# seanwood/gcc-nmf

Measured on AMD Instinct MI355X. Metric: stereo frames/sec (1024-FFT, K=1024, 100 NMF iters), higher is better.
Workload: dtype f32; 1 GPU; HBM-resident (float32 samples in HBM -> separated float32 waveforms in HBM; the host-to-host rates are the host_to_host_* fields of a --full run): 64 x 10 s stereo @16 kHz synthetic mixtures per GPU (SURVEY 8d recipe), 1024-pt FFT hop 256 (F=513, T=622/file), K=1024, 100 KL-NMF iters, 128 TDOAs, 3 targets, independent dictionary per file; dictionary_size=1024, parallelism=file-sharded x1, no data-path collective

## Files before the change

gcc_nmf_amd/csrc/common.h:

```cpp
#pragma once
#include <hip/hip_runtime.h>
#include <stdint.h>

#define GCCNMF_OK 0
#define GCCNMF_ERR_ARG 1
#define GCCNMF_ERR_LAUNCH 2
#define GCCNMF_ERR_UNSUPPORTED 3

static inline int gccnmf_ceil_div(int a, int b) { return (a + b - 1) / b; }
static inline int gccnmf_round_up(int a, int b) { return gccnmf_ceil_div(a, b) * b; }

#define GCCNMF_CHECK_LAUNCH()                                   \
    do {                                                        \
        hipError_t e__ = hipGetLastError();                     \
        if (e__ != hipSuccess) return GCCNMF_ERR_LAUNCH;        \
    } while (0)

struct GccNmfPitches {
    int Fp, Kp, Np, Tp;
};

static inline GccNmfPitches gccnmf_make_pitches(int F, int T, int K) {
    GccNmfPitches p;
    p.Fp = gccnmf_round_up(F, 16);
    p.Kp = gccnmf_round_up(K, 64);
    p.Np = gccnmf_round_up(2 * T, 64);
    p.Tp = gccnmf_round_up(T, 64);
    return p;
}

#define GCCNMF_TUNE_KEYS 26
struct GccNmfTune {
    int v[GCCNMF_TUNE_KEYS];
};
extern thread_local GccNmfTune gccnmf_tune;
struct GccNmfCall {
    GccNmfCall();
    ~GccNmfCall();
};
#define GCCNMF_ENTER() GccNmfCall gccnmf_call_scope_
#define gccnmf_tune_ablate (gccnmf_tune.v[1])
#define gccnmf_tune_tile_policy (gccnmf_tune.v[2])
#define gccnmf_tune_dma (gccnmf_tune.v[3])
#define gccnmf_tune_ring (gccnmf_tune.v[4])
#define gccnmf_tune_wh_splits (gccnmf_tune.v[5])
#define gccnmf_tune_rht_splits (gccnmf_tune.v[6])
#define gccnmf_tune_exact_div (gccnmf_tune.v[7])
#define gccnmf_tune_shared_groups (gccnmf_tune.v[8])
#define gccnmf_tune_tail_split (gccnmf_tune.v[9])
#define gccnmf_tune_direct (gccnmf_tune.v[10])
#define gccnmf_tune_direct_tile (gccnmf_tune.v[11])
#define gccnmf_tune_direct_batch (gccnmf_tune.v[12])
#define gccnmf_tune_direct_depth (gccnmf_tune.v[13])
#define gccnmf_tune_short_updh (gccnmf_tune.v[14])
#define gccnmf_tune_fft_r16 (gccnmf_tune.v[15])
#define gccnmf_tune_fused_k12 (gccnmf_tune.v[16])
#define gccnmf_tune_fused_k34 (gccnmf_tune.v[17])
#define gccnmf_tune_persistent (gccnmf_tune.v[18])
#define gccnmf_tune_prefetch (gccnmf_tune.v[19])
#define gccnmf_tune_wide_update_w (gccnmf_tune.v[20])
#define gccnmf_tune_chain (gccnmf_tune.v[21])
#define gccnmf_tune_chain_solo (gccnmf_tune.v[22])
#define gccnmf_tune_chain_rag (gccnmf_tune.v[23])
#define gccnmf_tune_chain_chunk (gccnmf_tune.v[24])
#define gccnmf_tune_chain_fault (gccnmf_tune.v[25])
```

gcc_nmf_amd/csrc/gcc.hip:

```cpp
#include "gemm_ring.h"
#include "ratio.h"
#include "spatial.h"
#include "angular_nl.h"
#include "atom_tdoa.h"
#include "source_count.h"
#include "../../include/gccnmf_hip.h"


static bool gcc_small_launch(int batch, int M, int N, int Kd) {
    if (!gccnmf_tune_ring || !gccnmf_ring_supports(Kd) || gccnmf_tune_tile_policy == 1) return false;
    if (gccnmf_tune_tile_policy == 2) return true;
    return (long)batch * gccnmf_ceil_div(M, 512) * gccnmf_ceil_div(N, 64) < 256;
}

__global__ __launch_bounds__(256) void ang_mean_kernel(const float* __restrict__ ang, int T, int D, int Dp, int Tp,
                                                       double* __restrict__ mean_ang) {
    __shared__ double red[256];
    const int b = blockIdx.x / D, d = blockIdx.x - b * D;
    const float* row = ang + ((long)b * Dp + d) * Tp;
    double s = 0.0;
    for (int t = threadIdx.x; t < T; t += 256) s += (double)row[t];
    red[threadIdx.x] = s;
    __syncthreads();
    for (int w = 128; w > 0; w >>= 1) {
// ... 150 lines not shown
        const float* sin_row = trig + ((long)Fp + f) * Dp;
        int4 tau;
        if (TRACKS) tau = *(const int4*)(tdoa_idx + ((long)b * S + i) * Tp + t);
        else tau.x = tau.y = tau.z = tau.w = tdoa_idx[(long)b * S + i];
        const bool absent = COUNTED && tau.x < 0;
        tau.x = tau.x < 0 ? 0 : (tau.x >= D ? D - 1 : tau.x);
        tau.y = tau.y < 0 ? 0 : (tau.y >= D ? D - 1 : tau.y);
        tau.z = tau.z < 0 ? 0 : (tau.z >= D ? D - 1 : tau.z);
        tau.w = tau.w < 0 ? 0 : (tau.w >= D ? D - 1 : tau.w);
        out = gcc_steer4(cr, ci, make_float4(cos_row[tau.x], cos_row[tau.y], cos_row[tau.z], cos_row[tau.w]),
                         make_float4(sin_row[tau.x], sin_row[tau.y], sin_row[tau.z], sin_row[tau.w]));
        if (absent) out.x = out.y = out.z = out.w = __builtin_nanf("");
        if (t + 1 >= T) out.y = 0.f;
        if (t + 2 >= T) out.z = 0.f;
        if (t + 3 >= T) out.w = 0.f;
    }
    *(float4*)(P + ((long)b * Fp + f) * ((long)S * Tp) + col) = out;
}

__global__ __launch_bounds__(256) void gcc_argmax_kernel(const float* __restrict__ scores, int K, int Kp, int T, int Tp, int S,
                                                         unsigned char* __restrict__ argmax) {
    const int t = 4 * (blockIdx.x * 256 + threadIdx.x);
    const int k = blockIdx.y, b = blockIdx.z;
    if (t >= Tp) return;
    unsigned char best[4] = {0, 0, 0, 0};
    if (k < K && t < T) {
        const float* row = scores + ((long)b * Kp + k) * ((long)S * Tp) + t;
        float bv[4] = {0.f, 0.f, 0.f, 0.f};
        bool have[4] = {false, false, false, false};
        for (int i = 0; i < S; ++i) {
            const float4 v4 = *(const float4*)(row + (long)i * Tp);
            const float v[4] = {v4.x, v4.y, v4.z, v4.w};
#pragma unroll
            for (int j = 0; j < 4; ++j) {
                if (v[j] != v[j]) continue;
                if (!have[j] || v[j] > bv[j]) {
                    bv[j] = v[j];
                    best[j] = (unsigned char)i;
                    have[j] = true;
                }
            }
        }
#pragma unroll
        for (int j = 1; j < 4; ++j)
            if (t + j >= T) best[j] = 0;
    }
    *(uchar4*)(argmax + ((long)b * Kp + k) * Tp + t) = make_uchar4(best[0], best[1], best[2], best[3]);
}

__global__ __launch_bounds__(256) void gcc_coherence_kernel(const float2* __restrict__ X, int Fp, int T, int Tp,
                                                            float* __restrict__ CC) {
    const int t = blockIdx.x * 256 + threadIdx.x;
    const int f = blockIdx.y, b = blockIdx.z;
    if (t >= T) return;
    const long plane = (long)Fp * Tp;
    const float2 xl = X[(long)b * 2 * plane + (long)f * Tp + t];
    const float2 xr = X[(long)b * 2 * plane + plane + (long)f * Tp + t];
    const float aL = hypotf(xl.x, xl.y), aR = hypotf(xr.x, xr.y);
    float re = xl.x * xr.x + xl.y * xr.y, im = xl.y * xr.x - xl.x * xr.y;
    if (aL > 0.f && aR > 0.f) {
        re = re / aL / aR;
        im = im / aL / aR;
    } else {
        re = 0.f;
        im = 0.f;
    }
    float* Cb = CC + (long)b * 2 * plane + (long)f * Tp + t;
    Cb[0] = re;
    Cb[plane] = im;
}

__global__ __launch_bounds__(256) void gcc_magnitude_kernel(const float2* __restrict__ X, int Fp, int T, int Tp, int Np,
                                                            float* __restrict__ V) {
    const int t = blockIdx.x * 256 + threadIdx.x;
    const int f = blockIdx.y, b = blockIdx.z >> 1, c = blockIdx.z & 1;
    if (t >= T) return;
    const float2 x = X[((long)b * 2 + c) * Fp * Tp + (long)f * Tp + t];
    V[(long)b * Fp * Np + (long)f * Np + c * T + t] = hypotf(x.x, x.y);
}

__global__ __launch_bounds__(256) void gcc_masked_h_kernel(const float* __restrict__ H, const unsigned char* __restrict__ argmax,
                                                           const float* __restrict__ masks, int K, int Kp, int T, int Tp, int Np,
                                                           int S, float* __restrict__ Hm) {
    const int col = 4 * (blockIdx.x * 256 + threadIdx.x);
    const int k = blockIdx.y, b = blockIdx.z;
    const int ncol = 2 * S * Tp;
    if (col >= ncol) return;
    const int ic = col / Tp, t = col - ic * Tp;
    const int i = ic >> 1, c = ic & 1;
    float4 out = make_float4(0.f, 0.f, 0.f, 0.f);
    if (k < K && t < T) {
        const float* h = H + ((long)b * Kp + k) * Np + c * T + t;
        float4 m;
        if (masks) {
            m = *(const float4*)(masks + (((long)b * S + i) * Kp + k) * Tp + t);
        } else {
            const uchar4 a = *(const uchar4*)(argmax + ((long)b * Kp + k) * Tp + t);
            m = make_float4(a.x == i ? 1.f : 0.f, a.y == i ? 1.f : 0.f, a.z == i ? 1.f : 0.f, a.w == i ? 1.f : 0.f);
        }
        out.x = h[0] * m.x;
        if (t + 1 < T) out.y = h[1] * m.y;
        if (t + 2 < T) out.z = h[2] * m.z;
        if (t + 3 < T) out.w = h[3] * m.w;
    }
    *(float4*)(Hm + ((long)b * Kp + k) * (long)ncol + col) = out;
}

int gccnmf_gemm_nn_store(const float* A, const float* B, float* C, int M, int N, int Kd, int lda, int ldb, int ldc, int batch, long sA,
                         long sB, long sC, hipStream_t s) {
    GemmArgs a = {};
    a.A = A; a.sA = sA; a.lda = lda; a.a_clamp = lda - 4;
    a.B = B; a.sB = sB; a.ldb = ldb; a.b_clamp = ldb - 4;
    a.M = M; a.N = N; a.Kd = Kd;
    a.batch = batch; a.xcd_affine = 0;
    a.C = C; a.sC = sC; a.ldc = ldc;
    if (gcc_small_launch(batch, a.M, a.N, a.Kd)) return gccnmf_launch_gemm_ring<false, false, EPI_STORE, false>(a, s);
    return (M > 128) ? gccnmf_launch_gemm<4, 1, false, false, EPI_STORE, false>(a, s) : gccnmf_launch_gemm<1, 4, false, false, EPI_STORE, false>(a, s);
}

extern "C" {

int gccnmf_angular_spectrogram(const float* CC, const float* trig, int F, int T, int D, int batch, float* ang,
                               double* mean_ang, void* stream) {
    GCCNMF_ENTER();
    const unsigned alpha_bits = ((unsigned)D & 0xffff0000u) | ((unsigned)batch >> 16);
    float nl_alpha = 0.f;
    if (alpha_bits) {
        __builtin_memcpy(&nl_alpha, &alpha_bits, sizeof(float));
        if (!gccnmf_nl_alpha_ok(nl_alpha)) return GCCNMF_ERR_ARG;
        D &= 0xffff;
        batch &= 0xffff;
    }
    if (!CC || !trig || !ang || F < 2 || T < 1 || D < 1 || batch < 1) return GCCNMF_ERR_ARG;
    hipStream_t s = (hipStream_t)stream;
    GccNmfPitches p = gccnmf_make_pitches(F, T, 1);
    const int Dp = gccnmf_round_up(D, 64);
    if (alpha_bits) {
        const int rc = gccnmf_launch_angular_nl(CC, trig, F, T, D, batch, nl_alpha, ang, s);
        if (rc) return rc;
        if (mean_ang) {
            hipLaunchKernelGGL(ang_mean_kernel, dim3(batch * D), dim3(256), 0, s, ang, T, D, Dp, p.Tp, mean_ang);
            GCCNMF_CHECK_LAUNCH();
        }
        return GCCNMF_OK;
    }
    GemmArgs a = {};
    a.A = trig; a.sA = 0; a.lda = Dp; a.a_clamp = Dp - 4;
    a.B = CC; a.sB = 2L * p.Fp * p.Tp; a.ldb = p.Tp; a.b_clamp = p.Tp - 4;
    a.M = D; a.N = T; a.Kd = 2 * p.Fp;
    a.batch = batch; a.xcd_affine = 0;
    a.C = ang; a.sC = (long)Dp * p.Tp; a.ldc = p.Tp;
    int rc;
    if (gcc_small_launch(batch, a.M, a.N, a.Kd)) rc = gccnmf_launch_gemm_ring<false, false, EPI_STORE, false>(a, s);
    else rc = (D > 128) ? gccnmf_launch_gemm<4, 1, false, false, EPI_STORE, false>(a, s)
                        : gccnmf_launch_gemm<1, 4, false, false, EPI_STORE, false>(a, s);
    if (rc) return rc;
    if (mean_ang) {
        hipLaunchKernelGGL(ang_mean_kernel, dim3(batch * D), dim3(256), 0, s, ang, T, D, Dp, p.Tp, mean_ang);
        GCCNMF_CHECK_LAUNCH();
    }
    return GCCNMF_OK;
}

int gccnmf_pick_tdoa_peaks(const double* mean_ang, int D, int Dp, int S, int batch, int* tdoa_idx, int* status,
                           void* stream) {
    GCCNMF_ENTER();
    if (S > 0 && (S & ~0xff) == GCCNMF_PEAKS_COUNT_BIT) {
        S &= 0xff;
        if (!mean_ang || !tdoa_idx || !status || D < 3 || D > SOURCE_COUNT_MAX_D || Dp < D || S < 1 || batch < 1) return GCCNMF_ERR_ARG;
        return gccnmf_launch_count_peaks(mean_ang, D, Dp, S, batch, tdoa_idx, status, (hipStream_t)stream);
    }
    if (S & ~0xff) {
        const int L = (S >> 9) & 0x3fffff, T = Dp;
        if (S < 0 || !(S & GCCNMF_PEAKS_TRACKS_BIT) || L < 1) return GCCNMF_ERR_ARG;
        S &= 0xff;
        if (!mean_ang || !tdoa_idx || !status || D < 3 || D > 4096 || T < 1 || T >= (1 << 21) || S < 1 || batch < 1 || batch > 65535)
            return GCCNMF_ERR_ARG;
        const int Tp = gccnmf_round_up(T, 64);
        hipLaunchKernelGGL(track_peaks_kernel, dim3(T, batch), dim3(64), 8 * D + 16 + gccnmf_round_up(D, 16), (hipStream_t)stream, (const float*)mean_ang, T, Tp, D,
                           gccnmf_round_up(D, 64), S, L, tdoa_idx, status);
        GCCNMF_CHECK_LAUNCH();
        hipLaunchKernelGGL(track_carry_kernel, dim3(batch), dim3(256), 0, (hipStream_t)stream, T, Tp, S, tdoa_idx, status);
        GCCNMF_CHECK_LAUNCH();
        return GCCNMF_OK;
    }
    if (!mean_ang || !tdoa_idx || !status || D < 3 || D > 4096 || Dp < D || S < 1 || batch < 1) return GCCNMF_ERR_ARG;
    hipLaunchKernelGGL(pick_peaks_kernel, dim3(batch), dim3(64), 0, (hipStream_t)stream, mean_ang, D, Dp, S, tdoa_idx, status);
    GCCNMF_CHECK_LAUNCH();
// ... 58 lines not shown
    }
    a.batch = batch; a.xcd_affine = 1;
    a.C = scores; a.sC = (long)p.Kp * ncol; a.ldc = ncol;
    int rc;
    if (gcc_small_launch(batch, a.M, a.N, a.Kd)) rc = gccnmf_launch_gemm_ring<false, false, EPI_STORE, false>(a, s);
    else if (K > 128 && gccnmf_tune_dma && gccnmf_tune_ablate != 128) rc = gccnmf_launch_gemm_dma<false, false, EPI_STORE, false>(a, s);
    else rc = (K > 128) ? gccnmf_launch_gemm<4, 1, false, false, EPI_STORE, false>(a, s)
                        : gccnmf_launch_gemm<1, 4, false, false, EPI_STORE, false>(a, s);
    if (rc) return rc;
    if (argmax) {
        hipLaunchKernelGGL(gcc_argmax_kernel, dim3(gccnmf_ceil_div(p.Tp, 1024), p.Kp, batch), dim3(256), 0, s, scores, K, p.Kp, T,
                           p.Tp, S, argmax);
        GCCNMF_CHECK_LAUNCH();
    }
    return GCCNMF_OK;
}

int gccnmf_argmax_targets(const float* scores, int K, int T, int S, int batch, unsigned char* argmax, void* stream) {
    GCCNMF_ENTER();
    if (!scores || !argmax || K < 1 || T < 1 || S < 1 || S > 255 || batch < 1) return GCCNMF_ERR_ARG;
    GccNmfPitches p = gccnmf_make_pitches(2, T, K);
    hipLaunchKernelGGL(gcc_argmax_kernel, dim3(gccnmf_ceil_div(p.Tp, 1024), p.Kp, batch), dim3(256), 0, (hipStream_t)stream, scores,
                       K, p.Kp, T, p.Tp, S, argmax);
    GCCNMF_CHECK_LAUNCH();
    return GCCNMF_OK;
}

int gccnmf_coherence(const float* X, int F, int T, int batch, float* CC, void* stream) {
    GCCNMF_ENTER();
    if (!X || !CC || F < 2 || T < 1 || batch < 1) return GCCNMF_ERR_ARG;
    GccNmfPitches p = gccnmf_make_pitches(F, T, 1);
    hipLaunchKernelGGL(gcc_coherence_kernel, dim3(gccnmf_ceil_div(T, 256), F, batch), dim3(256), 0, (hipStream_t)stream,
                       (const float2*)X, p.Fp, T, p.Tp, CC);
    GCCNMF_CHECK_LAUNCH();
    return GCCNMF_OK;
}

int gccnmf_magnitude(const float* X, int F, int T, int batch, float* V, void* stream) {
    GCCNMF_ENTER();
    if (!X || !V || F < 2 || T < 1 || batch < 1) return GCCNMF_ERR_ARG;
    GccNmfPitches p = gccnmf_make_pitches(F, T, 1);
    hipLaunchKernelGGL(gcc_magnitude_kernel, dim3(gccnmf_ceil_div(T, 256), F, batch * 2), dim3(256), 0, (hipStream_t)stream,
                       (const float2*)X, p.Fp, T, p.Tp, p.Np, V);
    GCCNMF_CHECK_LAUNCH();
    return GCCNMF_OK;
}

long gccnmf_reconstruct_workspace_floats(int T, int K, int S, int batch) {
    GCCNMF_ENTER();
    if (T < 1 || K < 1 || S < 1 || batch < 1) return -1;
    GccNmfPitches p = gccnmf_make_pitches(2, T, K);
    return (long)batch * p.Kp * 2 * S * p.Tp;
}

int gccnmf_reconstruct(const float* W, const float* H, const unsigned char* argmax, const float* masks, const float* X,
                       const float* V, int F, int T, int K, int S, int batch, float* workspace, float* spec, void* stream) {
    GCCNMF_ENTER();
    const int mode = S & ~0xff;
    S &= 0xff;
    if (mode & ~(GCCNMF_RECONSTRUCT_RATIO | GCCNMF_RECONSTRUCT_SPATIAL_ITERATIONS(0xff))) return GCCNMF_ERR_ARG;
    const bool ratio = (mode & GCCNMF_RECONSTRUCT_RATIO) != 0;
    const int iterations = (mode >> 20) & 0xff;
    if (batch < 1 || (batch & ~(0xffff | GCCNMF_RECONSTRUCT_SPATIAL_BIT))) return GCCNMF_ERR_ARG;
    const bool spatial = (batch & GCCNMF_RECONSTRUCT_SPATIAL_BIT) != 0;
    batch &= 0xffff;
    if (spatial && !ratio) return GCCNMF_ERR_ARG;
    if (iterations && !spatial) return GCCNMF_ERR_ARG;
    if (!W || !H || (!argmax && !masks) || !X || (!ratio && (!V || !workspace)) || !spec || F < 2 || T < 1 || K < 1 || S < 1 || batch < 1)
        return GCCNMF_ERR_ARG;
    if (spatial && (!workspace || ((uintptr_t)workspace & 15))) return GCCNMF_ERR_ARG;
    if (ratio && S > GCCNMF_RATIO_MAX_TARGETS) return GCCNMF_ERR_UNSUPPORTED;
    hipStream_t s = (hipStream_t)stream;
    if (ratio) {
        const int rc = gccnmf_launch_ratio(W, H, argmax, masks, X, F, T, K, S, batch, spec, s);
        if (rc != GCCNMF_OK || !spatial) return rc;
        if (!iterations) return gccnmf_launch_spatial(X, F, T, S, batch, workspace, spec, s);
        GccNmfPitches p = gccnmf_make_pitches(F, T, 1);
        float* powers = workspace + GCCNMF_RECONSTRUCT_SPATIAL_WORKSPACE_FLOATS(batch, S, p.Fp);
        return gccnmf_launch_spatial_em(X, F, T, S, batch, iterations, workspace, powers, spec, s);
    }
    GccNmfPitches p = gccnmf_make_pitches(F, T, K);
    const int ncol = 2 * S * p.Tp;
    float* Hm = workspace;
    hipLaunchKernelGGL(gcc_masked_h_kernel, dim3(gccnmf_ceil_div(ncol, 1024), p.Kp, batch), dim3(256), 0, s, H, argmax, masks, K, p.Kp,
                       T, p.Tp, p.Np, S, Hm);
    GCCNMF_CHECK_LAUNCH();
    const bool tail = (F % 128) == 1;
    GemmArgs a = {};
    a.A = W; a.sA = (long)p.Fp * p.Kp; a.lda = p.Kp; a.a_clamp = p.Fp - 1;
    a.B = Hm; a.sB = (long)p.Kp * ncol; a.ldb = ncol; a.b_clamp = ncol - 4;
    a.M = tail ? F - 1 : F; a.N = ncol; a.Kd = K;
    a.tail_row = F - 1;
    a.batch = batch; a.xcd_affine = 1;
    a.C = spec; a.sC = 2L * S * p.Fp * p.Tp;
    a.E0 = V; a.sE0 = (long)p.Fp * p.Np;
    a.X = (const float2*)X; a.sX = 2L * p.Fp * p.Tp;
    a.T = T; a.Tp = p.Tp; a.Fp = p.Fp; a.ldv = p.Np;
    if (gcc_small_launch(batch, a.M, a.N, a.Kd))
        return tail ? gccnmf_launch_gemm_ring<true, false, EPI_PHASE, true>(a, s) : gccnmf_launch_gemm_ring<true, false, EPI_PHASE, false>(a, s);
    const bool tall = a.M > 128;
    if (tall && gccnmf_tune_dma && gccnmf_tune_ablate != 128)
        return tail ? gccnmf_launch_gemm_dma<true, false, EPI_PHASE, true>(a, s) : gccnmf_launch_gemm_dma<true, false, EPI_PHASE, false>(a, s);
    if (tall) return tail ? gccnmf_launch_gemm<4, 1, true, false, EPI_PHASE, true>(a, s)
                          : gccnmf_launch_gemm<4, 1, true, false, EPI_PHASE, false>(a, s);
    return tail ? gccnmf_launch_gemm<1, 4, true, false, EPI_PHASE, true>(a, s)
                : gccnmf_launch_gemm<1, 4, true, false, EPI_PHASE, false>(a, s);
}

}
```

gcc_nmf_amd/csrc/gemm_dma.h:

```cpp
#pragma once
#include <mutex>
#include <type_traits>
#include "gemm_mfma.h"
#include "chain_sync.h"

#ifndef GEMM_DMA_ABL
#define GEMM_DMA_ABL 0
#endif

typedef __attribute__((address_space(3))) void* gemm_lds_ptr;
typedef __attribute__((address_space(1))) const void* gemm_glb_ptr;

__device__ __forceinline__ void gemm_dma16(const float* wave_uniform_base, unsigned lane_byte_offset, unsigned lds_wave_byte_addr) {
    asm volatile("s_mov_b32 m0, %2\n\tglobal_load_lds_dwordx4 %0, %1"
                 :
                 : "v"(lane_byte_offset), "s"(wave_uniform_base), "s"(lds_wave_byte_addr)
                 : "memory");
}

__device__ __forceinline__ void gemm_dma16_masked(const float* wave_uniform_base, unsigned lane_byte_offset, unsigned lds_wave_byte_addr,
                                                  unsigned long long wave_uniform_mask) {
    unsigned long long saved;
    asm volatile("s_mov_b64 %0, exec\n\ts_mov_b64 exec, %4\n\ts_mov_b32 m0, %3\n\tglobal_load_lds_dwordx4 %1, %2\n\ts_mov_b64 exec, %0"
                 : "=&s"(saved)
// ... 103 lines not shown
#pragma unroll
        for (int e = 0; e < 4; ++e)
#pragma unroll
            for (int h = 0; h < NT / 2; ++h) v[e][h] *= s[e];
    }
};

__device__ __forceinline__ float gemm_div_fast(float v, float d) {
    const float r = __builtin_amdgcn_rcpf(d);
    const float q = v * r;
    return fmaf(fmaf(-d, q, v), r, q);
}

typedef int gemm_i32x4 __attribute__((ext_vector_type(4)));
__device__ float gemm_buffer_load(gemm_i32x4 rsrc, int voffset, int soffset, int aux) __asm("llvm.amdgcn.raw.buffer.load.f32");
__device__ gemm_f32x4 gemm_buffer_load4(gemm_i32x4 rsrc, int voffset, int soffset, int aux) __asm("llvm.amdgcn.raw.buffer.load.v4f32");
__device__ void gemm_buffer_store(float data, gemm_i32x4 rsrc, int voffset, int soffset, int aux) __asm("llvm.amdgcn.raw.buffer.store.f32");
__device__ __forceinline__ gemm_i32x4 gemm_buffer_rsrc(const void* wave_uniform_base, long bytes = 0x7fffffffL) {
    const unsigned long long a = (unsigned long long)wave_uniform_base;
    gemm_i32x4 r;
    r.x = __builtin_amdgcn_readfirstlane((int)(unsigned)a);
    r.y = __builtin_amdgcn_readfirstlane((int)(unsigned)(a >> 32) & 0xffff);
    r.z = __builtin_amdgcn_readfirstlane((int)(bytes < 0x7fffffffL ? bytes : 0x7fffffffL));
    r.w = 0x00020000;
    return r;
}

template <int EPI, int BM = 512>
struct GemmEpiloguePair {
    static_assert(EPI == EPI_STORE || EPI == EPI_DIV || EPI == EPI_UPDH, "");
    float xa[16], xb[16];

    __device__ __forceinline__ void load(const GemmArgs& p, int file, int row_u, int hh, int col_a, long cb) {
        if (EPI == EPI_DIV || EPI == EPI_UPDH) {
            const int lo = 4 * (4 * hh * p.ldc + col_a);
            const int ro = 4 * row_u * p.ldc, rstep = 4 * p.ldc;
            const gemm_i32x4 X = gemm_buffer_rsrc(EPI == EPI_DIV ? p.E0 + file * p.sE0 : p.C + file * p.sC, cb);
#pragma unroll
            for (int r = 0; r < 16; ++r) {
                const int so = ro + ((r & 3) + 8 * (r >> 2)) * rstep;
                xa[r] = gemm_buffer_load(X, lo, so, 0);
                xb[r] = gemm_buffer_load(X, lo + 128, so, 0);
            }
        }
    }

    __device__ __forceinline__ void finish(const GemmArgs& p, int file, int row_u, int tile_row, int hh, int col_a, float ba, float bb,
                                           const float* s_rowvec, const f32x16& acc_a, const f32x16& acc_b, bool oka, bool okb, long cb) const {
        const int lo = 4 * (4 * hh * p.ldc + col_a);
        const int ro = 4 * row_u * p.ldc, rstep = 4 * p.ldc;
        const gemm_i32x4 C = gemm_buffer_rsrc(p.C + file * p.sC, cb);
        auto column = [&](const f32x16& acc, const float (&x)[16], const float b, const int lane_off) {
            float u[16];
#pragma unroll
            for (int r = 0; r < 16; ++r) u[r] = acc[r];
            if (EPI == EPI_STORE || EPI == EPI_UPDH) {
#pragma unroll
                for (int g = 0; g < 4; ++g) {
                    const gemm_f32x4 tav = *(const gemm_f32x4*)(s_rowvec + tile_row + 8 * g + 4 * hh);
                    gemm_f32x4 gv = {1.f, 1.f, 1.f, 1.f};
                    if (EPI == EPI_UPDH) gv = *(const gemm_f32x4*)(s_rowvec + BM + tile_row + 8 * g + 4 * hh);
#pragma unroll
                    for (int i = 0; i < 4; ++i) {
                        const int r = 4 * g + i;
                        u[r] = fmaf(tav[i], b, u[r]);
                        if (EPI == EPI_UPDH) u[r] = (x[r] * u[r]) * gv[i];
                    }
                }
            }
            if (EPI == EPI_DIV) {
                if (p.exact_div) {
#pragma unroll
                    for (int r = 0; r < 16; ++r) u[r] = x[r] / u[r];
                } else {
#pragma unroll
                    for (int r = 0; r < 16; ++r) u[r] = gemm_div_fast(x[r], u[r]);
                }
            }
#pragma unroll
            for (int r = 0; r < 16; ++r) gemm_buffer_store(u[r], C, lane_off, ro + ((r & 3) + 8 * (r >> 2)) * rstep, 0);
        };
        if (oka) column(acc_a, xa, ba, lo);
        if (okb) column(acc_b, xb, bb, lo + 128);
    }
};

template <bool TAIL>
__device__ __forceinline__ void gemm_epilogue_update_w_full(const GemmArgs& p, int file, int col0, int tid, int wm, int l31, int hh,
                                                            bool wave_active, f32x16 (&acc)[4][2], float tail_acc, float rowsum_acc,
                                                            float* smem) {
    float* s_rs = smem;
    float* s_tail = smem + 64;
    float* s_red = smem + 320;
    float* s_norm = smem + 640;
    float rs = rowsum_acc;
    rs += __shfl_xor(rs, 1);
    rs += __shfl_xor(rs, 2);
    if ((tid & 3) == 0) s_rs[tid >> 2] = rs;
    if (TAIL) s_tail[tid] = tail_acc;
    __syncthreads();
    const int ca = l31, cb = l31 + 32;
    const float ira = 1.0f / s_rs[ca], irb = 1.0f / s_rs[cb];
    const gemm_i32x4 W = gemm_buffer_rsrc(p.C + file * p.sC);
    const int lo = 4 * (4 * hh * p.ldc + col0 + l31), rstep = 4 * p.ldc;
    float ssa = 0.f, ssb = 0.f;
    if (wave_active) {
#pragma unroll
        for (int m = 0; m < 4; ++m) {
            const int ro = (wm * 128 + m * 32) * rstep;
            float wa[16], wb[16];
#pragma unroll
            for (int r = 0; r < 16; ++r) {
                const int so = ro + ((r & 3) + 8 * (r >> 2)) * rstep;
                wa[r] = gemm_buffer_load(W, lo, so, 0);
                wb[r] = gemm_buffer_load(W, lo + 128, so, 0);
            }
#pragma unroll
            for (int r = 0; r < 16; ++r) {
                const float ta = wa[r] * (acc[m][0][r] * ira), tb = wb[r] * (acc[m][1][r] * irb);
                acc[m][0][r] = ta;
                acc[m][1][r] = tb;
                ssa = fmaf(ta, ta, ssa);
                ssb = fmaf(tb, tb, ssb);
            }
        }
    }
    ssa += __shfl_xor(ssa, 32);
    ssb += __shfl_xor(ssb, 32);
    if (hh == 0) {
        s_red[wm * 64 + ca] = ssa;
        s_red[wm * 64 + cb] = ssb;
    }
    float wt_tail = 0.f;
    float* Wp = p.C + file * p.sC;
    if (tid < 64) {
        if (TAIL) {
            const float u = (s_tail[tid] + s_tail[64 + tid]) + (s_tail[128 + tid] + s_tail[192 + tid]);
            wt_tail = Wp[(long)p.tail_row * p.ldc + col0 + tid] * (u / s_rs[tid]);
        }
        s_red[256 + tid] = wt_tail * wt_tail;
    }
    __syncthreads();
    if (tid < 64) s_norm[tid] = sqrtf(((s_red[tid] + s_red[64 + tid]) + (s_red[128 + tid] + s_red[192 + tid])) + s_red[256 + tid]);
    __syncthreads();
    const float ina = 1.0f / s_norm[ca], inb = 1.0f / s_norm[cb];
    float csa = 0.f, csb = 0.f;
    if (wave_active) {
#pragma unroll
        for (int m = 0; m < 4; ++m) {
            const int ro = (wm * 128 + m * 32) * rstep;
#pragma unroll
            for (int r = 0; r < 16; ++r) {
                const int so = ro + ((r & 3) + 8 * (r >> 2)) * rstep;
                const float na = acc[m][0][r] * ina, nb = acc[m][1][r] * inb;
                gemm_buffer_store(na, W, lo, so, 0);
                gemm_buffer_store(nb, W, lo + 128, so, 0);
                csa += na;
                csb += nb;
            }
        }
    }
    csa += __shfl_xor(csa, 32);
    csb += __shfl_xor(csb, 32);
    if (hh == 0) {
        s_red[wm * 64 + ca] = csa;
        s_red[wm * 64 + cb] = csb;
// ... 478 lines not shown
#pragma unroll
            for (int n = 0; n < 2; ++n)
#pragma unroll
                for (int r = 0; r < 16; ++r) acc[m][n][r] = 0.f;
        tail_acc = 0.f;
        rowsum_acc = 0.f;
        if constexpr (EPI == EPI_STORE || EPI == EPI_UPDH) {
#pragma unroll
            for (int i = 0; i < BM / 256; ++i) {
                const int lr = tid + 256 * i, row = min(row0 + lr, p.M - 1);
                s_rowvec[lr] = p.ktailA ? p.ktailA[file * p.s_ktailA + row] : 0.f;
                if (EPI == EPI_UPDH) {
                    const float rd = 1.0f / (p.E2[file * p.sE2 + row] + p.alpha + p.eps);
                    s_rowvec[BM + lr] = p.E1 ? p.E1[file * p.sE1 + row] * rd : rd;
                }
            }
        }
        if (tid == 0) {
            s_arrivals = 0;
            if (persistent) s_ticket[it & 1] = p.wpl + (int)__hip_atomic_fetch_add(p.tickets + list, 1u, __ATOMIC_RELAXED, __HIP_MEMORY_SCOPE_AGENT);
        }
        asm volatile("s_waitcnt vmcnt(0)" ::: "memory");
        __syncthreads();
        read_group0(lds0);
        wait_group0();

        if constexpr (NARROW) {
            if (nw == 1) main_loop(std::integral_constant<int, 1>{});
            else main_loop(std::integral_constant<int, 2>{});
        } else {
            main_loop(std::integral_constant<int, 2>{});
        }
        __syncthreads();
        if (trace_row && tid == 0) trace_row[2] = __builtin_amdgcn_s_memrealtime();

        const int e_file = file, e_row0 = row0, e_col0 = col0, e_nw = nw, e_n = n_item;
        const bool e_active = wave_active, e_tail = do_tail, e_rowsum = do_rowsum;
        have = false;
        prefetched = false;
        if (persistent) {
            t = __builtin_amdgcn_readfirstlane(s_ticket[it & 1]);
            have = take_item(t);
            if (have && p.prefetch) {
                set_offsets(gemm_opaque_tid() & 63);
#pragma unroll
                for (int i = 0; i < NPIECES; ++i) dma_piece(i, 0, 0);
                prefetched = true;
            }
        }
        float* const scratch = smem + SBUF;

        if constexpr (EPI == EPI_UPDW) {
            if constexpr (TM == 4) gemm_epilogue_update_w_full<TAIL>(p, e_file, e_col0, tid, wm, l31, hh, e_active, acc, tail_acc, rowsum_acc, scratch);
        } else {
            if (e_active) {
                const int row_w = e_row0 + wm * RW;
                bool lean = false;
                if constexpr (EPI == EPI_STORE || EPI == EPI_DIV || EPI == EPI_UPDH) {
                    lean = row_w + RW <= p.M;
                    if (lean) {
                        GemmEpiloguePair<EPI, BM> e0, e1;
                        const int ca = e_col0 + l31, tr = wm * RW;
                        const bool oka = ca < e_n, okb = (!NARROW || e_nw == 2) && ca + 32 < e_n;
                        const long cb = 4L * p.ldc * (p.M + (TAIL ? 1 : 0));
                        float ba = 0.f, bb = 0.f;
                        e0.load(p, e_file, row_w, hh, ca, cb);
                        e1.load(p, e_file, row_w + 32, hh, ca, cb);
                        if (EPI != EPI_DIV && p.ktailA) {
                            ba = p.ktailB[e_file * p.s_ktailB + min(ca, e_n - 1)];
                            bb = p.ktailB[e_file * p.s_ktailB + min(ca + 32, e_n - 1)];
                        }
                        e0.finish(p, e_file, row_w, tr, hh, ca, ba, bb, s_rowvec, acc[0][0], acc[0][1], oka, okb, cb);
                        if (trace_row && tid == 0) trace_row[5] = __builtin_amdgcn_s_memrealtime();
                        if constexpr (TM == 4) e0.load(p, e_file, row_w + 64, hh, ca, cb);
                        e1.finish(p, e_file, row_w + 32, tr + 32, hh, ca, ba, bb, s_rowvec, acc[1][0], acc[1][1], oka, okb, cb);
                        if constexpr (TM == 4) {
                            e1.load(p, e_file, row_w + 96, hh, ca, cb);
                            e0.finish(p, e_file, row_w + 64, tr + 64, hh, ca, ba, bb, s_rowvec, acc[2][0], acc[2][1], oka, okb, cb);
                            e1.finish(p, e_file, row_w + 96, tr + 96, hh, ca, ba, bb, s_rowvec, acc[3][0], acc[3][1], oka, okb, cb);
                        }
                        if (trace_row && tid == 0) trace_row[6] = __builtin_amdgcn_s_memrealtime();
                    }
                }
                if (!lean) {
                    GemmArgs pq = p;
                    pq.N = e_n;
#pragma unroll
                    for (int m = 0; m < TM; ++m)
                        gemm_epilogue_pair<EPI>(pq, e_file, row_w + m * 32 + 4 * hh, e_col0 + wn * 64 + l31, acc[m][0], acc[m][1], !NARROW || e_nw == 2);
                }
            }
            if (TAIL) {
                if (e_tail) {
                    scratch[tid] = tail_acc;
                    __syncthreads();
                    if (tid < (NARROW && e_nw == 1 ? 32 : BN)) {
                        const float s = (scratch[tid] + scratch[BN + tid]) + (scratch[2 * BN + tid] + scratch[3 * BN + tid]);
                        const int col = e_col0 + tid;
                        if (EPI == EPI_PHASE ? gemm_col_valid<EPI>(p, col) : col < e_n) gemm_epilogue<EPI>(p, e_file, p.tail_row, col, s);
                    }
                }
            }
            if (B_KC) {
                if (e_rowsum) {
                    float s = rowsum_acc;
                    s += __shfl_xor(s, 1);
                    s += __shfl_xor(s, 2);
                    const int j = tid >> 2;
                    if ((tid & 3) == 0 && (e_col0 + j) < e_n && (!NARROW || e_nw == 2 || j < 32)) p.rowsumB[e_file * p.s_rowsumB + e_col0 + j] = s;
                }
            }
        }
        if (trace_row) {
            asm volatile("s_waitcnt vmcnt(0)" ::: "memory");
            __syncthreads();
            if (tid == 0) trace_row[3] = __builtin_amdgcn_s_memrealtime();
        }
        gemm_sync_signal(sync, e_file, e_col0, e_nw, tid);
        ++it;
        if (have) __syncthreads();
    }
#ifdef GEMM_DMA_PROBE
    if (p.trace && lane == 0 && (long)p.trace_grid + 4L * blockIdx.x + 4 <= p.trace_rows) {
#pragma unroll
        for (int i = 0; i < 7; ++i) p.trace[8 * ((long)p.trace_grid + blockIdx.x * 4 + wave) + i] = (long long)probe[i];
        p.trace[8 * ((long)p.trace_grid + blockIdx.x * 4 + wave) + 7] = it;
    }
#endif
    if (persistent && tid == 0) {
        const unsigned gone = __hip_atomic_fetch_add(p.tickets + 8, 1u, __ATOMIC_ACQ_REL, __HIP_MEMORY_SCOPE_AGENT);
        if (gone == gridDim.x - 1) {
#pragma unroll
            for (int i = 0; i < 9; ++i) __hip_atomic_store(p.tickets + i, 0u, __ATOMIC_RELAXED, __HIP_MEMORY_SCOPE_AGENT);
        }
    }
}

template <bool A_KC, bool B_KC, int EPI, bool TAIL, int TM, bool NARROW>
__global__ __launch_bounds__(256, 2) void gccnmf_gemm_dma_kernel(GemmArgs p) {
    __shared__ __attribute__((aligned(16))) float smem[2 * GemmDmaLds<TM>::SBUF];
    __shared__ __attribute__((aligned(16))) float s_rowvec[(EPI == EPI_STORE || EPI == EPI_UPDH) ? 2 * 128 * TM : 4];
    __shared__ unsigned s_arrivals;
    __shared__ int s_ticket[2];
    const int list = p.lists == 8 ? (int)(blockIdx.x & 7) : 0;
    const int t = p.lists == 8 ? (int)(blockIdx.x >> 3) : (int)blockIdx.x;
    GemmSync none = {};
    gemm_dma_workgroup<A_KC, B_KC, EPI, TAIL, TM, NARROW>(p, smem, s_rowvec, &s_arrivals, s_ticket, list, t, none);
}

struct GemmChain {
    int first[5];
    int it0, iterations;
    int trace_it;
    GemmSync sync[4];
};
template <bool TAIL, int STAGES, int TM1>
__global__ __launch_bounds__(256, 2) void gccnmf_gemm_chain_kernel(GemmArgs p0, GemmArgs p1, GemmArgs p2, GemmArgs p3, GemmChain ch) {
    static_assert(STAGES == 2 || STAGES == 4, "");
    __shared__ __attribute__((aligned(16))) float smem[2 * GemmDmaLds<4>::SBUF];
    __shared__ __attribute__((aligned(16))) float s_rowvec[2 * 512];
    __shared__ unsigned s_arrivals;
    __shared__ int s_ticket[2];
    const int list = (int)(blockIdx.x & 7);
    int pos = (int)(blockIdx.x >> 3), it = ch.it0;
    if (ch.iterations > 1) {
        const int q = pos / ch.first[4];
// ... 122 lines not shown
```

gcc_nmf_amd/csrc/gemm_mfma.h:

```cpp
#pragma once
#include "common.h"

typedef float f32x16 __attribute__((ext_vector_type(16)));

#ifndef GEMM_VARIANT
#define GEMM_VARIANT 2
#endif
#if GEMM_VARIANT & 1
#define GEMM_PRIO(x) __builtin_amdgcn_s_setprio(x)
#else
#define GEMM_PRIO(x)
#endif
#if GEMM_VARIANT & 2
#define GEMM_PIN()
#else
#define GEMM_PIN() __builtin_amdgcn_sched_barrier(0)
#endif

extern long long* gccnmf_trace_buf;
extern int gccnmf_trace_blocks;

enum GemmEpilogue {
    EPI_STORE = 0,
    EPI_DIV = 1,
    EPI_UPDH = 2,
    EPI_PHASE = 3,
    EPI_UPDW = 4
};

#define GEMM_RAGGED_LMAX 31

struct GemmArgs {
    const float* A;
    const float* B;
    long sA, sB;
    int lda, ldb;
    int M, N, Kd;
    int a_clamp, b_clamp;
    int tiles_m, tiles_n, batch, xcd_affine;
    int concurrent;
    int file0;
    int kparts;
    int exact_div;
    int ablate;
    const float* bscale;
    long s_bscale;
    int tail_row;
    const float* ktailA;
    const float* ktailB;
    long s_ktailA, s_ktailB;
    float* out_colsum;
    float* out_norm;
    long s_out;
    float* rowsumB;
    long s_rowsumB;
    float* C;
    long sC;
    int ldc;
    const float* E0;
    long sE0;
    const float* E1;
    long sE1;
    const float* E2;
    long sE2;
    const float2* X;
    long sX;
    float alpha, eps;
    int T, Tp, Fp, ldv;
    long long* trace;
    int lists;
    int cw, cr;
    int split;
    int rag, wide_n;
    int whole_files;
    const int* ragged_n;
    const int* ragged_lists;
    int ragged_kd;
    int narrow_ok;
    int wpl, prefetch;
    unsigned* tickets;
    int trace_rows, trace_grid;
};

template <int EPI>
__device__ __forceinline__ bool gemm_col_valid(const GemmArgs& p, int col) {
    if (EPI == EPI_PHASE) {
        int ic = col / p.Tp;
        return col < p.N && (col - ic * p.Tp) < p.T;
    }
    return col < p.N;
}

template <int EPI>
__device__ __forceinline__ void gemm_epilogue(const GemmArgs& p, int file, int row, int col, float acc) {
    if (EPI == EPI_STORE) {
        p.C[file * p.sC + (long)row * p.ldc + col] = acc;
    } else if (EPI == EPI_DIV) {
        long idx = (long)row * p.ldc + col;
        p.C[file * p.sC + idx] = p.E0[file * p.sE0 + idx] / acc;
    } else if (EPI == EPI_UPDH) {
        long idx = file * p.sC + (long)row * p.ldc + col;
        float h = p.C[idx];
        if (p.E1) h *= p.E1[file * p.sE1 + row];
        float den = p.E2[file * p.sE2 + row] + p.alpha + p.eps;
        p.C[idx] = h * (acc / den);
    } else {
        int ic = col / p.Tp;
        int t = col - ic * p.Tp;
        int c = ic & 1;
        float2 x = p.X[file * p.sX + ((long)c * p.Fp + row) * p.Tp + t];
        float v = p.E0[file * p.sE0 + (long)row * p.ldv + c * p.T + t];
        float2 ph;
        if (v > 0.f) {
            ph.x = x.x / v;
            ph.y = x.y / v;
        } else {
            ph.x = 1.f;
            ph.y = 0.f;
        }
        float2 o;
        o.x = acc * ph.x;
        o.y = acc * ph.y;
        ((float2*)p.C)[file * p.sC + ((long)ic * p.Fp + row) * p.Tp + t] = o;
    }
}

template <int EPI>
__device__ __forceinline__ void gemm_epilogue_pair(const GemmArgs& p, int file, int row_base, int col_a, const f32x16& acc_in_a,
                                                   const f32x16& acc_in_b, bool allow_b = true) {
    const int col_b = col_a + 32;
    const bool ok_a = gemm_col_valid<EPI>(p, col_a), ok_b = allow_b && gemm_col_valid<EPI>(p, col_b);
    float acc_a[16], acc_b[16];
#pragma unroll
    for (int r = 0; r < 16; ++r) {
        acc_a[r] = acc_in_a[r];
        acc_b[r] = acc_in_b[r];
    }
    if (EPI == EPI_STORE || EPI == EPI_UPDH) {
        if (p.ktailA) {
            const float* __restrict__ ta = p.ktailA + file * p.s_ktailA;
            const float* __restrict__ tb = p.ktailB + file * p.s_ktailB;
            const float ba = tb[min(col_a, p.N - 1)], bb = tb[min(col_b, p.N - 1)];
            float av[16];
#pragma unroll
            for (int r = 0; r < 16; ++r) av[r] = ta[min(row_base + (r & 3) + 8 * (r >> 2), p.M - 1)];
#pragma unroll
            for (int r = 0; r < 16; ++r) {
                acc_a[r] = fmaf(av[r], ba, acc_a[r]);
                acc_b[r] = fmaf(av[r], bb, acc_b[r]);
            }
        }
    }
    if (EPI == EPI_STORE) {
        float* __restrict__ C = p.C + file * p.sC;
#pragma unroll
        for (int r = 0; r < 16; ++r) {
            const int row = row_base + (r & 3) + 8 * (r >> 2);
            if (row < p.M) {
                if (ok_a) C[(long)row * p.ldc + col_a] = acc_a[r];
                if (ok_b) C[(long)row * p.ldc + col_b] = acc_b[r];
            }
        }
    } else if (EPI == EPI_DIV) {
        const float* __restrict__ V = p.E0 + file * p.sE0;
// ... 483 lines not shown
```

gcc_nmf_amd/csrc/nmf.hip:

```cpp
#include <mutex>
#include "gemm_ring.h"
#include "direct.h"
#include "update_w.h"
#include "divergence.h"
#ifdef GCCNMF_EXPERIMENTS
int gccnmf_launch_gemm_stream(GemmArgs a, hipStream_t stream);
#endif
int gccnmf_klnmf_fixed_launch(const float* V, const float* W, float* H, float* workspace, int F, int N, int K, int batch, int iterations,
                              float alpha, float eps, bool ones, hipStream_t s);
bool gccnmf_klnmf_fixed_supported(int F, int K);
long gccnmf_klnmf_fixed_workspace_floats(int F, int K);
bool gccnmf_klnmf_semi_supported(int F, int K, int nfree);
int gccnmf_klnmf_semi_rht_launch(const float* R, const float* H, float* U, float* rowsumH, int F, int N, int K, int nfree, int batch, hipStream_t s);
int gccnmf_klnmf_semi_update_w_launch(float* W, const float* U, const float* rowsumH, float* colsumW, float* hscale, int F, int K, int nfree,
                                      int batch, hipStream_t s);
bool gccnmf_klnmf_beta_supported(int F, int K);
int gccnmf_klnmf_beta_stage_launch(int stage, int divergence, const float* V, float* W, float* H, float* R, float* Q, float* Un, float* Ud,
                                   float* colsumW, float* hscale, int F, int N, int K, int batch, float alpha, float eps, hipStream_t s);
#include "../../include/gccnmf_hip.h"

#include <atomic>
#include <algorithm>
#include <vector>
#define GCCNMF_SHARED_STREAMS 4
#define GCCNMF_CHAIN_MAX_ITERATIONS gccnmf_tune_chain_chunk
#define GCCNMF_RAGGED_MAX_BATCH 248
#define GCCNMF_SPLITS 4
#define GCCNMF_DIRECT_MAX_BATCH 8
struct GccNmfKnob {
    int def, lo, hi, experiment;
};
static const GccNmfKnob gccnmf_knobs[GCCNMF_TUNE_KEYS] = {
    {0, 0, 0, 1},
    {0, 0, 1 << 30, 1},
    {0, 0, 2, 0},
    {1, 0, 1, 0},
    {1, 0, 1, 1},
    {3, 1, 4, 1},
    {4, 1, 4, 1},
    {1, 0, 1, 0},
    {3, 1, GCCNMF_SHARED_STREAMS, 0},
    {1, 0, 3, 0},
    {1, 0, 1, 0},
    {0, 0, 8, 1},
    {4, 1, GCCNMF_DIRECT_MAX_BATCH, 0},
    {0, 0, 4, 1},
    {1, 0, 1, 1},
    {1, 0, 1, 1},
    {1, 0, 2, 0},
    {1, 0, 2, 0},
    {0, 0, 1, 1},
    {1, 0, 1, 1},
    {1, 0, 1, 1},
    {1, 0, 8, 0},
    {0, 0, 1, 1},
    {1, 0, 3, 0},
    {2048, 1, 65536, 0},
    {0, 0, 1, 1},
};
static std::atomic<int> gccnmf_knob_value[GCCNMF_TUNE_KEYS];
static std::atomic<int> gccnmf_knobs_ready{0};
static void gccnmf_knobs_init() {
    static std::mutex mu;
    if (gccnmf_knobs_ready.load(std::memory_order_acquire)) return;
    std::lock_guard<std::mutex> lock(mu);
    if (gccnmf_knobs_ready.load(std::memory_order_relaxed)) return;
    for (int k = 0; k < GCCNMF_TUNE_KEYS; ++k) gccnmf_knob_value[k].store(gccnmf_knobs[k].def, std::memory_order_relaxed);
    gccnmf_knobs_ready.store(1, std::memory_order_release);
}
static GccNmfTune gccnmf_tune_load() {
    gccnmf_knobs_init();
    GccNmfTune t;
    for (int k = 0; k < GCCNMF_TUNE_KEYS; ++k) t.v[k] = gccnmf_knob_value[k].load(std::memory_order_relaxed);
    return t;
}
thread_local GccNmfTune gccnmf_tune = gccnmf_tune_load();
static thread_local int gccnmf_call_depth = 0;
GccNmfCall::GccNmfCall() {
    if (gccnmf_call_depth++ == 0) gccnmf_tune = gccnmf_tune_load();
}
GccNmfCall::~GccNmfCall() { --gccnmf_call_depth; }
long long* gccnmf_trace_buf = nullptr;
int gccnmf_trace_blocks = 0;

extern "C" {
int gccnmf_version(void) { return 106; }

int gccnmf_set_tuning(int key, int value) {
    GCCNMF_ENTER();
    gccnmf_knobs_init();
    if (key < 1 || key >= GCCNMF_TUNE_KEYS) return GCCNMF_ERR_ARG;
    const GccNmfKnob& k = gccnmf_knobs[key];
#ifndef GCCNMF_EXPERIMENTS
    if (k.experiment) return GCCNMF_ERR_ARG;
#endif
    if (value < k.lo || value > k.hi || (key == 13 && value == 1) || (key == 21 && value != 0 && value != 1 && value != 2 && value != 4 && value != 8)) return GCCNMF_ERR_ARG;
    gccnmf_knob_value[key].store(value, std::memory_order_relaxed);
    return GCCNMF_OK;
}

}

#ifdef GCCNMF_EXPERIMENTS
unsigned* gccnmf_ticket_block(hipStream_t stream) {
    constexpr int MAX_DEV = 16, PER_DEV = 128;
    struct Entry { hipStream_t s; };
    static std::mutex mu;
    static unsigned* pool[MAX_DEV] = {};
    static Entry entries[MAX_DEV][PER_DEV];
    static int used[MAX_DEV] = {};
    int dev = 0;
    if (hipGetDevice(&dev) != hipSuccess || dev < 0 || dev >= MAX_DEV) return nullptr;
    std::lock_guard<std::mutex> lock(mu);
    for (int i = 0; i < used[dev]; ++i)
        if (entries[dev][i].s == stream) return pool[dev] + 16 * i;
    if (used[dev] == PER_DEV) return nullptr;
    if (!pool[dev]) {
        static const unsigned zeros[16 * PER_DEV] = {};
        unsigned* p = nullptr;
        if (hipMalloc((void**)&p, sizeof(zeros)) != hipSuccess) {
            (void)hipGetLastError();
            return nullptr;
        }
        if (hipMemcpy(p, zeros, sizeof(zeros), hipMemcpyHostToDevice) != hipSuccess) {
            (void)hipGetLastError();
            (void)hipFree(p);
            return nullptr;
        }
        pool[dev] = p;
    }
    entries[dev][used[dev]].s = stream;
    return pool[dev] + 16 * used[dev]++;
}

#endif

extern "C" {
#ifdef GCCNMF_EXPERIMENTS
int gccnmf_debug_set_trace(long long* buf, int blocks) {
    GCCNMF_ENTER();
    gccnmf_trace_buf = buf;
// ... 1421 lines not shown
```

Before: 157,100 frames/s.

## Batch phase-epilogue loads with buffer ops and restructure masked-H kernel per atom-time

Adds a new phase-reconstruction epilogue path in the DMA GEMM that loads X and V tiles with raw buffer loads, ahead of use and interleaved across row tiles, then writes complex outputs with buffer stores. It is guarded by a new knob that defaults on. The masked-H kernel is also reorganised so each thread reads H and the argmax once and writes all source/channel columns, cutting redundant reads. The trade is higher register pressure from staging 16 complex values per tile, plus a new code path whose correctness depends on the addressability check.

```diff
diff --git a/gcc_nmf_amd/csrc/common.h b/gcc_nmf_amd/csrc/common.h
--- a/gcc_nmf_amd/csrc/common.h
+++ b/gcc_nmf_amd/csrc/common.h
@@ -29,7 +29,7 @@
     return p;
 }
 
-#define GCCNMF_TUNE_KEYS 26
+#define GCCNMF_TUNE_KEYS 27
 struct GccNmfTune {
     int v[GCCNMF_TUNE_KEYS];
 };
@@ -64,3 +64,4 @@
 #define gccnmf_tune_chain_rag (gccnmf_tune.v[23])
 #define gccnmf_tune_chain_chunk (gccnmf_tune.v[24])
 #define gccnmf_tune_chain_fault (gccnmf_tune.v[25])
+#define gccnmf_tune_phase_batched (gccnmf_tune.v[26])
diff --git a/gcc_nmf_amd/csrc/gcc.hip b/gcc_nmf_amd/csrc/gcc.hip
--- a/gcc_nmf_amd/csrc/gcc.hip
+++ b/gcc_nmf_amd/csrc/gcc.hip
@@ -256,28 +256,47 @@
 __global__ __launch_bounds__(256) void gcc_masked_h_kernel(const float* __restrict__ H, const unsigned char* __restrict__ argmax,
                                                            const float* __restrict__ masks, int K, int Kp, int T, int Tp, int Np,
                                                            int S, float* __restrict__ Hm) {
-    const int col = 4 * (blockIdx.x * 256 + threadIdx.x);
-    const int k = blockIdx.y, b = blockIdx.z;
-    const int ncol = 2 * S * Tp;
-    if (col >= ncol) return;
-    const int ic = col / Tp, t = col - ic * Tp;
-    const int i = ic >> 1, c = ic & 1;
-    float4 out = make_float4(0.f, 0.f, 0.f, 0.f);
-    if (k < K && t < T) {
-        const float* h = H + ((long)b * Kp + k) * Np + c * T + t;
+    const int q = Tp >> 2;
+    const int idx = blockIdx.x * 256 + threadIdx.x;
+    const int b = blockIdx.y;
+    if (idx >= Kp * q) return;
+    const int k = idx / q, t = 4 * (idx - k * q);
+    const long ncol = 2L * S * Tp;
+    float* out = Hm + ((long)b * Kp + k) * ncol + t;
+    if (k >= K || t >= T) {
+        const float4 zero = make_float4(0.f, 0.f, 0.f, 0.f);
+        for (int ic = 0; ic < 2 * S; ++ic) *(float4*)(out + (long)ic * Tp) = zero;
+        return;
+    }
+    const float* h = H + ((long)b * Kp + k) * Np + t;
+    const bool v1 = t + 1 < T, v2 = t + 2 < T, v3 = t + 3 < T;
+    float4 hc[2];
+    hc[0] = *(const float4*)h;
+    if ((T & 3) == 0) {
+        hc[1] = *(const float4*)(h + T);
+    } else {
+        hc[1].x = h[T];
+        hc[1].y = v1 ? h[T + 1] : 0.f;
+        hc[1].z = v2 ? h[T + 2] : 0.f;
+        hc[1].w = v3 ? h[T + 3] : 0.f;
+    }
+    uchar4 a = make_uchar4(0, 0, 0, 0);
+    if (!masks) a = *(const uchar4*)(argmax + ((long)b * Kp + k) * Tp + t);
+    for (int i = 0; i < S; ++i) {
         float4 m;
-        if (masks) {
+        if (masks)
             m = *(const float4*)(masks + (((long)b * S + i) * Kp + k) * Tp + t);
-        } else {
-            const uchar4 a = *(const uchar4*)(argmax + ((long)b * Kp + k) * Tp + t);
+        else
             m = make_float4(a.x == i ? 1.f : 0.f, a.y == i ? 1.f : 0.f, a.z == i ? 1.f : 0.f, a.w == i ? 1.f : 0.f);
-        }
-        out.x = h[0] * m.x;
-        if (t + 1 < T) out.y = h[1] * m.y;
-        if (t + 2 < T) out.z = h[2] * m.z;
-        if (t + 3 < T) out.w = h[3] * m.w;
-    }
-    *(float4*)(Hm + ((long)b * Kp + k) * (long)ncol + col) = out;
+#pragma unroll
+        for (int c = 0; c < 2; ++c) {
+            float4 o = make_float4(hc[c].x * m.x, 0.f, 0.f, 0.f);
+            if (v1) o.y = hc[c].y * m.y;
+            if (v2) o.z = hc[c].z * m.z;
+            if (v3) o.w = hc[c].w * m.w;
+            *(float4*)(out + (long)(2 * i + c) * Tp) = o;
+        }
+    }
 }
 
 int gccnmf_gemm_nn_store(const float* A, const float* B, float* C, int M, int N, int Kd, int lda, int ldb, int ldc, int batch, long sA,
@@ -502,7 +521,7 @@
     GccNmfPitches p = gccnmf_make_pitches(F, T, K);
     const int ncol = 2 * S * p.Tp;
     float* Hm = workspace;
-    hipLaunchKernelGGL(gcc_masked_h_kernel, dim3(gccnmf_ceil_div(ncol, 1024), p.Kp, batch), dim3(256), 0, s, H, argmax, masks, K, p.Kp,
+    hipLaunchKernelGGL(gcc_masked_h_kernel, dim3(gccnmf_ceil_div(p.Kp * (p.Tp / 4), 256), batch), dim3(256), 0, s, H, argmax, masks, K, p.Kp,
                        T, p.Tp, p.Np, S, Hm);
     GCCNMF_CHECK_LAUNCH();
     const bool tail = (F % 128) == 1;
@@ -516,6 +535,7 @@
     a.E0 = V; a.sE0 = (long)p.Fp * p.Np;
     a.X = (const float2*)X; a.sX = 2L * p.Fp * p.Tp;
     a.T = T; a.Tp = p.Tp; a.Fp = p.Fp; a.ldv = p.Np;
+    a.phase_batched = gccnmf_tune_phase_batched;
     if (gcc_small_launch(batch, a.M, a.N, a.Kd))
         return tail ? gccnmf_launch_gemm_ring<true, false, EPI_PHASE, true>(a, s) : gccnmf_launch_gemm_ring<true, false, EPI_PHASE, false>(a, s);
     const bool tall = a.M > 128;
diff --git a/gcc_nmf_amd/csrc/gemm_dma.h b/gcc_nmf_amd/csrc/gemm_dma.h
--- a/gcc_nmf_amd/csrc/gemm_dma.h
+++ b/gcc_nmf_amd/csrc/gemm_dma.h
@@ -209,6 +209,48 @@
         };
         if (oka) column(acc_a, xa, ba, lo);
         if (okb) column(acc_b, xb, bb, lo + 128);
+    }
+};
+
+__device__ gemm_f32x2 gemm_buffer_load2(gemm_i32x4 rsrc, int voffset, int soffset, int aux) __asm("llvm.amdgcn.raw.buffer.load.v2f32");
+__device__ void gemm_buffer_store2(gemm_f32x2 data, gemm_i32x4 rsrc, int voffset, int soffset, int aux) __asm("llvm.amdgcn.raw.buffer.store.v2f32");
+struct GemmEpiloguePhaseTile {
+    gemm_f32x2 x[16];
+    float v[16];
+
+    static __device__ __forceinline__ bool addressable(const GemmArgs& p) { return (long)p.Fp * max(2 * p.Tp, p.ldv) < (1L << 28); }
+
+    __device__ __forceinline__ void load(const GemmArgs& p, int file, int ic, int row_u, int hh, int t) {
+        const int c = ic & 1;
+        const gemm_i32x4 X = gemm_buffer_rsrc(p.X + file * p.sX + (long)c * p.Fp * p.Tp, 8L * p.Fp * p.Tp);
+        const gemm_i32x4 V = gemm_buffer_rsrc(p.E0 + file * p.sE0, 4L * p.Fp * p.ldv);
+        const int lx = 8 * (4 * hh * p.Tp + t), lv = 4 * (4 * hh * p.ldv + c * p.T + t);
+#pragma unroll
+        for (int r = 0; r < 16; ++r) {
+            const int row = row_u + (r & 3) + 8 * (r >> 2);
+            x[r] = gemm_buffer_load2(X, lx, 8 * p.Tp * row, 0);
+            v[r] = gemm_buffer_load(V, lv, 4 * p.ldv * row, 0);
+        }
+    }
+
+    __device__ __forceinline__ void finish(const GemmArgs& p, int file, int ic, int row_u, int hh, int t, const f32x16& acc, bool ok) const {
+        const gemm_i32x4 C = gemm_buffer_rsrc((const float2*)p.C + file * p.sC + (long)ic * p.Fp * p.Tp, 8L * p.Fp * p.Tp);
+        const int lx = 8 * (4 * hh * p.Tp + t);
+        gemm_f32x2 o[16];
+#pragma unroll
+        for (int r = 0; r < 16; ++r) {
+            const float a = acc[r];
+            float qx = x[r].x / v[r], qy = x[r].y / v[r];
+            asm volatile("" : "+v"(qx), "+v"(qy));
+            const bool some = v[r] > 0.f;
+            o[r].x = some ? a * qx : a;
+            o[r].y = some ? a * qy : 0.f;
+            asm volatile("" : "+v"(o[r]));
+        }
+        if (ok) {
+#pragma unroll
+            for (int r = 0; r < 16; ++r) gemm_buffer_store2(o[r], C, lx, 8 * p.Tp * (row_u + (r & 3) + 8 * (r >> 2)), 0);
+        }
     }
 };
 
@@ -853,6 +895,23 @@
                         if (trace_row && tid == 0) trace_row[6] = __builtin_amdgcn_s_memrealtime();
                     }
                 }
+                if constexpr (EPI == EPI_PHASE) {
+                    lean = p.phase_batched && row_w + RW <= p.M && GemmEpiloguePhaseTile::addressable(p);
+                    if (lean) {
+                        GemmEpiloguePhaseTile ea, eb;
+                        const int ic = e_col0 / p.Tp, ta = e_col0 - ic * p.Tp + l31, tb = ta + 32;
+                        const bool oka = ta < p.T, okb = tb < p.T;
+                        ea.load(p, e_file, ic, row_w, hh, ta);
+                        eb.load(p, e_file, ic, row_w, hh, tb);
+#pragma unroll
+                        for (int m = 0; m < TM; ++m) {
+                            ea.finish(p, e_file, ic, row_w + 32 * m, hh, ta, acc[m][0], oka);
+                            if (m + 1 < TM) ea.load(p, e_file, ic, row_w + 32 * (m + 1), hh, ta);
+                            eb.finish(p, e_file, ic, row_w + 32 * m, hh, tb, acc[m][1], okb);
+                            if (m + 1 < TM) eb.load(p, e_file, ic, row_w + 32 * (m + 1), hh, tb);
+                        }
+                    }
+                }
                 if (!lean) {
                     GemmArgs pq = p;
                     pq.N = e_n;
diff --git a/gcc_nmf_amd/csrc/gemm_mfma.h b/gcc_nmf_amd/csrc/gemm_mfma.h
--- a/gcc_nmf_amd/csrc/gemm_mfma.h
+++ b/gcc_nmf_amd/csrc/gemm_mfma.h
@@ -80,6 +80,7 @@
     int wpl, prefetch;
     unsigned* tickets;
     int trace_rows, trace_grid;
+    int phase_batched;
 };
 
 template <int EPI>
diff --git a/gcc_nmf_amd/csrc/nmf.hip b/gcc_nmf_amd/csrc/nmf.hip
--- a/gcc_nmf_amd/csrc/nmf.hip
+++ b/gcc_nmf_amd/csrc/nmf.hip
@@ -57,6 +57,7 @@
     {1, 0, 3, 0},
     {2048, 1, 65536, 0},
     {0, 0, 1, 1},
+    {1, 0, 1, 0},
 };
 static std::atomic<int> gccnmf_knob_value[GCCNMF_TUNE_KEYS];
 static std::atomic<int> gccnmf_knobs_ready{0};
```

Result: no change. 157,200 frames/s (median of 4 runs) (+0.1%).
